# theblackcat102/edgedict

Measured on AMD Instinct MI355X. Metric: utterances/sec (E6D2, 15 s audio), higher is better.
Workload: dtype bf16; 1 GPU; E6D2 full training step (dither+log-mel+stack3+SpecAugment masks -> 6x1024 LSTM encoder, 2x time reduction -> 2x256 LSTM prediction net -> joint 640 -> RNN-T loss -> backward -> grad all-reduce -> Adam); 64 x 15 s utterances per GPU, U=64, V=2048, ragged lengths; lattice [64,201,65,2048]; global_batch=64, parallelism=dp1

## Files before the change

### edgedict_amd/config.py

```python
import os

import torch

_NAMES = {"fp32": torch.float32, "float32": torch.float32, "f32": torch.float32,
          "bf16": torch.bfloat16, "bfloat16": torch.bfloat16}


def _parse(x):
    if isinstance(x, torch.dtype):
        if x not in (torch.float32, torch.bfloat16):
            raise ValueError("compute dtype must be float32 or bfloat16")
        return x
    try:
        return _NAMES[str(x).lower()]
    except KeyError:
        raise ValueError("unknown compute dtype %r (use 'fp32' or 'bf16')" % (x,))


FORCE_GENERIC_LSTM = False

USE_ENCODER_STACK = os.environ.get("EDGEDICT_ENCODER_STACK", "1") != "0"

DEFER_WEIGHT_GRADS = os.environ.get("EDGEDICT_DEFER_DW", "1") != "0"
FUSED_DB2 = os.environ.get("EDGEDICT_FUSED_DB2", "1") != "0"

DECODER_ON_AUX_STREAM = os.environ.get("EDGEDICT_DECODER_AUX", "1") != "0"

DECODER_ENQUEUE_FIRST = os.environ.get("EDGEDICT_DECODER_FIRST", "0") != "0"

PACKED_LATTICE = os.environ.get("EDGEDICT_PACKED_LATTICE", "1") != "0"

FUSED_LSE = os.environ.get("EDGEDICT_FUSED_LSE", "1") != "0"

BAND_LATTICE = os.environ.get("EDGEDICT_BAND_LATTICE", "0") != "0"

STREAM_ENCODER_STEP = os.environ.get("EDGEDICT_STREAM_ENCODER_STEP", "1") != "0"
STREAM_STEP_MAX_ROWS_SHORT = int(os.environ.get("EDGEDICT_STREAM_STEP_MAX_ROWS_SHORT", "4096"))
STREAM_FAST_CHUNK = os.environ.get("EDGEDICT_STREAM_FAST_CHUNK", "1") != "0"
STREAM_STEP_MAX_ROWS = int(os.environ.get("EDGEDICT_STREAM_STEP_MAX_ROWS", "16"))

STACK_MIN_FRAMES = int(os.environ.get("EDGEDICT_STACK_MIN_FRAMES", "24"))

_state = {"dtype": _parse(os.environ.get("EDGEDICT_DTYPE", "fp32")), "epoch": 0}


def set_compute_dtype(x):
    _state["dtype"] = _parse(x)


def get_compute_dtype():
    return _state["dtype"]


def bump_param_epoch():
    _state["epoch"] += 1


def param_epoch():
    return _state["epoch"]
```

### edgedict_amd/csrc/elementwise.hip

```cpp
#include <cstdlib>
#include "common.hpp"

namespace {

template <typename TS, typename TD>
__global__ void cast_kernel(const TS* __restrict__ s, TD* __restrict__ d, long long n) {
    for (long long i = (long long)blockIdx.x * blockDim.x + threadIdx.x; i < n;
         i += (long long)gridDim.x * blockDim.x)
        ElemIO<TD>::store(d + i, ElemIO<TS>::load(s + i));
}

template <typename TS, typename TD>
__global__ __launch_bounds__(256) void transpose_kernel(const TS* __restrict__ s,
                                                        TD* __restrict__ d, int R, int C) {
    __shared__ float tile[32][33];
    const int tx = threadIdx.x & 31, ty = threadIdx.x >> 5;
    const int c0 = blockIdx.x * 32, r0 = blockIdx.y * 32;
#pragma unroll
    for (int i = 0; i < 4; ++i) {
        const int r = r0 + ty + i * 8, c = c0 + tx;
        tile[ty + i * 8][tx] = (r < R && c < C) ? ElemIO<TS>::load(s + (long long)r * C + c) : 0.f;
    }
    __syncthreads();
#pragma unroll
// ... 311 lines not shown
#pragma unroll
            for (int e = 0; e < 8; ++e) usum[i][e] = 0.f;
        for (int t = t0 + wave; t < t1; t += 4) {
            const int lo = max(0, bd[2 * t]), hi = min(U1 - 1, bd[2 * t + 1]);
            const long long r0 = ro[t];
            const bool ok = hi >= lo && r0 >= 0 && r0 + (hi - lo) < rows;
            const long long base = (r0 - lo) * J + j0;
            float tsum[8] = {0.f, 0.f, 0.f, 0.f, 0.f, 0.f, 0.f, 0.f};
#pragma unroll
            for (int i = 0; i < JB_NU; ++i) {
                const int u = ubase + uc + ug + 8 * i;
                if (ok && u >= lo && u <= hi && jlive) {
                    float h[8], g[8];
                    Load8<T>::ld(hid + base + (long long)u * J, h);
                    Load8<T>::ld(dhid + base + (long long)u * J, g);
#pragma unroll
                    for (int e = 0; e < 8; ++e) {
                        const float dp = g[e] * (1.f - h[e] * h[e]);
                        tsum[e] += dp;
                        usum[i][e] += dp;
                    }
                }
            }
#pragma unroll
            for (int e = 0; e < 8; ++e) {
                tsum[e] += __shfl_xor(tsum[e], 8, 64);
                tsum[e] += __shfl_xor(tsum[e], 16, 64);
                tsum[e] += __shfl_xor(tsum[e], 32, 64);
            }
            if (ug == 0 && jlive) {
                float* de = dE1 + ((long long)b * Tn + t) * J + j0;
                if (uc == 0) {
                    *reinterpret_cast<float4*>(de) = make_float4(tsum[0], tsum[1], tsum[2], tsum[3]);
                    *reinterpret_cast<float4*>(de + 4) = make_float4(tsum[4], tsum[5], tsum[6], tsum[7]);
                } else {
#pragma unroll
                    for (int e = 0; e < 8; ++e) de[e] += tsum[e];
                }
            }
        }
        if (span <= 0) break;
        if (uc > 0) __syncthreads();
        if (wave >= 2) {
#pragma unroll
            for (int i = 0; i < JB_NU; ++i) {
                red[wave - 2][i][0][lane] = make_float4(usum[i][0], usum[i][1], usum[i][2], usum[i][3]);
                red[wave - 2][i][1][lane] = make_float4(usum[i][4], usum[i][5], usum[i][6], usum[i][7]);
            }
        }
        __syncthreads();
        if (wave < 2) {
#pragma unroll
            for (int i = 0; i < JB_NU; ++i) {
                const float4 p = red[wave][i][0][lane], q = red[wave][i][1][lane];
                usum[i][0] += p.x; usum[i][1] += p.y; usum[i][2] += p.z; usum[i][3] += p.w;
                usum[i][4] += q.x; usum[i][5] += q.y; usum[i][6] += q.z; usum[i][7] += q.w;
            }
        }
        __syncthreads();
        if (wave == 1) {
#pragma unroll
            for (int i = 0; i < JB_NU; ++i) {
                red[0][i][0][lane] = make_float4(usum[i][0], usum[i][1], usum[i][2], usum[i][3]);
                red[0][i][1][lane] = make_float4(usum[i][4], usum[i][5], usum[i][6], usum[i][7]);
            }
        }
        __syncthreads();
        if (wave == 0 && jlive) {
#pragma unroll
            for (int i = 0; i < JB_NU; ++i) {
                const int u = ubase + uc + ug + 8 * i;
                if (u > uend) continue;
                const float4 p = red[0][i][0][lane], q = red[0][i][1][lane];
                float* dd = dD1 + ((long long)b * U1 + u) * J + j0;
                atomicAdd(dd + 0, usum[i][0] + p.x); atomicAdd(dd + 1, usum[i][1] + p.y);
                atomicAdd(dd + 2, usum[i][2] + p.z); atomicAdd(dd + 3, usum[i][3] + p.w);
                atomicAdd(dd + 4, usum[i][4] + q.x); atomicAdd(dd + 5, usum[i][5] + q.y);
                atomicAdd(dd + 6, usum[i][6] + q.z); atomicAdd(dd + 7, usum[i][7] + q.w);
            }
        }
    }
}

__global__ void adam_kernel(float* __restrict__ p, const float* __restrict__ g,
                            float* __restrict__ m, float* __restrict__ v, long long n, float lr,
                            float b1, float b2, float omb1, float omb2, float eps, float bc1, float bc2,
                            float weight_decay, float grad_scale_host,
                            const float* __restrict__ grad_scale,
                            bf16_t* __restrict__ p_bf16, const unsigned* __restrict__ skip) {
    if (skip && *skip != 0u) return;
    const float gs = grad_scale_host * (grad_scale ? *grad_scale : 1.f);
    const float step = lr / bc1;
    const float inv_sqrt_bc2 = rsqrtf(bc2);
    for (long long i = (long long)blockIdx.x * blockDim.x + threadIdx.x; i < n;
         i += (long long)gridDim.x * blockDim.x) {
        float gi = g[i] * gs;
        float pi = p[i];
        if (weight_decay != 0.f) gi += weight_decay * pi;
        const float mi = b1 * m[i] + omb1 * gi;
        const float vi = b2 * v[i] + omb2 * gi * gi;
        m[i] = mi;
        v[i] = vi;
        pi -= step * mi / (sqrtf(vi) * inv_sqrt_bc2 + eps);
        p[i] = pi;
        if (p_bf16) p_bf16[i] = f32_to_bf16(pi);
    }
}

__global__ void guard_fetch_kernel(const unsigned* words, int n, unsigned* scratch) {
    if (threadIdx.x == 0) {
        unsigned any = 0u;
        for (int k = 0; k < n; ++k) any |= __hip_atomic_load(words + k, __ATOMIC_RELAXED, __HIP_MEMORY_SCOPE_SYSTEM);
        *scratch = any;
    }
}

__global__ __launch_bounds__(256) void sumsq_kernel(const float* __restrict__ x, long long n,
                                                    float* __restrict__ out) {
    __shared__ float part[4];
    float a = 0.f;
    for (long long i = (long long)blockIdx.x * blockDim.x + threadIdx.x; i < n;
         i += (long long)gridDim.x * blockDim.x)
        a += x[i] * x[i];
    a = wave_sum(a);
    if ((threadIdx.x & 63) == 0) part[threadIdx.x >> 6] = a;
    __syncthreads();
    if (threadIdx.x == 0) atomicAdd(out, part[0] + part[1] + part[2] + part[3]);
}
__global__ void clip_coef_kernel(const float* sumsq, float max_norm, float pre_scale, float* coef,
                                 float* norm_out) {
    const float nrm = sqrtf(*sumsq) * pre_scale;
    if (norm_out) *norm_out = nrm;
    *coef = fminf(1.f, max_norm / (nrm + 1e-6f));
}

template <typename T>
__global__ __launch_bounds__(256) void log_softmax_rows_kernel(const T* __restrict__ x, long long ldx,
                                                               float* __restrict__ y, int N) {
    const int r = blockIdx.x, tid = threadIdx.x, lane = tid & 63, wave = tid >> 6;
    const T* xr = x + (long long)r * ldx;
    __shared__ float part[4];
    float m = -INFINITY;
    for (int i = tid; i < N; i += 256) m = fmaxf(m, ElemIO<T>::load(xr + i));
    m = wave_max(m);
    if (lane == 0) part[wave] = m;
    __syncthreads();
    m = fmaxf(fmaxf(part[0], part[1]), fmaxf(part[2], part[3]));
    __syncthreads();
    float se = 0.f;
    for (int i = tid; i < N; i += 256) se += expf(ElemIO<T>::load(xr + i) - m);
    se = wave_sum(se);
    if (lane == 0) part[wave] = se;
    __syncthreads();
    const float logs = logf((part[0] + part[1]) + (part[2] + part[3]));
    float* yr = y + (long long)r * N;
    for (int i = tid; i < N; i += 256) yr[i] = (ElemIO<T>::load(xr + i) - m) - logs;
}
template <typename T>
__global__ __launch_bounds__(256) void log_softmax_rows_bwd_kernel(const float* __restrict__ y,
                                                                   const float* __restrict__ dy, long long lddy,
                                                                   T* __restrict__ dx, int N) {
    const int r = blockIdx.x, tid = threadIdx.x, lane = tid & 63, wave = tid >> 6;
    const float* yr = y + (long long)r * N;
    const float* dyr = dy + (long long)r * lddy;
    __shared__ float part[4];
    float a = 0.f;
// ... 172 lines not shown
    if (B == 0 || T == 0 || (n_t == 0 && n_f == 0)) return ED_OK;
    ED_CHECK_ARG(x, "spec_mask: null pointer");
    hipLaunchKernelGGL(spec_mask_kernel, dim3(ed_grid_for((long long)B * T * F, 256 * 4, 256 * 16)),
                       dim3(256), 0, (hipStream_t)stream_, x, B, T, F, t_iv, n_t, f_iv, n_f);
    ED_CHECK_LAUNCH("spec_mask");
    return ED_OK;
}

static int joint_hidden_fwd_impl(int dtype, const void* E1, const void* D1, void* hid, int B, int T,
                                 int U1, int J, const int32_t* act_lens, const int32_t* label_lens,
                                 const long long* pk_off, void* stream_) {
    ED_CHECK_ARG(dtype == ED_F32 || dtype == ED_BF16, "joint_hidden_fwd: bad dtype");
    ED_CHECK_ARG(B > 0 && T > 0 && U1 > 0 && J > 0, "joint_hidden_fwd: bad shape");
    const int vec = dtype == ED_F32 ? 4 : 8;
    ED_CHECK_ARG(J % vec == 0, "joint_hidden_fwd: joint size %d must be a multiple of %d", J, vec);
    ED_CHECK_ARG(E1 && D1 && hid, "joint_hidden_fwd: null pointer");
    hipStream_t s = (hipStream_t)stream_;
    ED_CHECK_ARG(J / vec <= 256, "joint_hidden_fwd: joint size %d too large", J);
    const int grid = ed_grid_for((long long)B * T, 1, 256 * 64);
    if (dtype == ED_F32)
        hipLaunchKernelGGL(joint_hidden_fwd<float>, dim3(grid), dim3(256), 0, s, (const float*)E1, (const float*)D1, (float*)hid, B, T, U1, J, act_lens, label_lens, pk_off);
    else
        hipLaunchKernelGGL(joint_hidden_fwd<bf16_t>, dim3(grid), dim3(256), 0, s, (const bf16_t*)E1, (const bf16_t*)D1, (bf16_t*)hid, B, T, U1, J, act_lens, label_lens, pk_off);
    ED_CHECK_LAUNCH("joint_hidden_fwd");
    return ED_OK;
}

extern "C" int edgedict_joint_hidden_fwd(int dtype, const void* E1, const void* D1, void* hid,
                                         int B, int T, int U1, int J, void* stream_) {
    return joint_hidden_fwd_impl(dtype, E1, D1, hid, B, T, U1, J, nullptr, nullptr, nullptr, stream_);
}

extern "C" int edgedict_joint_hidden_fwd_packed(int dtype, const void* E1, const void* D1, void* hid,
                                                const int32_t* act_lens, const int32_t* label_lens,
                                                const long long* row_offsets, int B, int T, int U1,
                                                int J, void* stream_) {
    ED_CHECK_ARG(act_lens && label_lens && row_offsets, "joint_hidden_fwd_packed: null lengths/offsets");
    return joint_hidden_fwd_impl(dtype, E1, D1, hid, B, T, U1, J, act_lens, label_lens, row_offsets, stream_);
}

static int joint_hidden_bwd_impl(int dtype, const void* dhid, const void* hid, float* dE1, float* dD1,
                                 int B, int T, int U1, int J, const int32_t* act_lens,
                                 const int32_t* label_lens, const long long* pk_off, void* stream_) {
    ED_CHECK_ARG(dtype == ED_F32 || dtype == ED_BF16, "joint_hidden_bwd: bad dtype");
    ED_CHECK_ARG(B > 0 && T > 0 && U1 > 0 && J > 0, "joint_hidden_bwd: bad shape");
    ED_CHECK_ARG(dhid && hid && dE1 && dD1, "joint_hidden_bwd: null pointer");
    hipStream_t s = (hipStream_t)stream_;
    hipError_t e = hipMemsetAsync(dD1, 0, (size_t)B * U1 * J * sizeof(float), s);
    if (e != hipSuccess) {
        ed_set_error("joint_hidden_bwd: memset failed: %s", hipGetErrorString(e));
        return ED_ERR_LAUNCH;
    }
    ED_CHECK_ARG(J % 8 == 0, "joint_hidden_bwd: joint size %d must be a multiple of 8", J);
    const int jblocks = (J + 63) / 64;
    static const int wg_target = [] { const char* e = getenv("EDGEDICT_JHB_WGS"); return e && atoi(e) > 0 ? atoi(e) : 1280; }();
    int tslabs = (wg_target + B * jblocks - 1) / (B * jblocks);
    if (tslabs > (T + 7) / 8) tslabs = (T + 7) / 8;
    if (tslabs < 1) tslabs = 1;
    const int tpb = (T + tslabs - 1) / tslabs;
    tslabs = (T + tpb - 1) / tpb;
    dim3 grid(jblocks, B, tslabs);
    if (dtype == ED_F32)
        hipLaunchKernelGGL(joint_hidden_bwd<float>, grid, dim3(256), 0, s, (const float*)dhid, (const float*)hid, dE1, dD1, B, T, U1, J, tpb, act_lens, label_lens, pk_off);
    else
        hipLaunchKernelGGL(joint_hidden_bwd<bf16_t>, grid, dim3(256), 0, s, (const bf16_t*)dhid, (const bf16_t*)hid, dE1, dD1, B, T, U1, J, tpb, act_lens, label_lens, pk_off);
    ED_CHECK_LAUNCH("joint_hidden_bwd");
    return ED_OK;
}

extern "C" int edgedict_joint_hidden_bwd(int dtype, const void* dhid, const void* hid, float* dE1,
                                         float* dD1, int B, int T, int U1, int J, void* stream_) {
    return joint_hidden_bwd_impl(dtype, dhid, hid, dE1, dD1, B, T, U1, J, nullptr, nullptr, nullptr, stream_);
}

extern "C" int edgedict_joint_hidden_bwd_packed(int dtype, const void* dhid, const void* hid,
                                                float* dE1, float* dD1, const int32_t* act_lens,
                                                const int32_t* label_lens,
                                                const long long* row_offsets, int B, int T, int U1,
                                                int J, void* stream_) {
    ED_CHECK_ARG(act_lens && label_lens && row_offsets, "joint_hidden_bwd_packed: null lengths/offsets");
    return joint_hidden_bwd_impl(dtype, dhid, hid, dE1, dD1, B, T, U1, J, act_lens, label_lens, row_offsets, stream_);
}

extern "C" int edgedict_joint_hidden_fwd_band(int dtype, const void* E1, const void* D1, void* hid, const int32_t* band,
                                              const long long* row_off, long long rows, int B, int T, int U1, int J,
                                              void* stream_) {
    ED_CHECK_ARG(dtype == ED_F32 || dtype == ED_BF16, "joint_hidden_fwd_band: bad dtype");
    ED_CHECK_ARG(B > 0 && T > 0 && U1 > 0 && J > 0 && rows >= 0, "joint_hidden_fwd_band: bad shape");
    const int vec = dtype == ED_F32 ? 4 : 8;
    ED_CHECK_ARG(J % vec == 0, "joint_hidden_fwd_band: joint size %d must be a multiple of %d", J, vec);
    ED_CHECK_ARG(J / vec <= 256, "joint_hidden_fwd_band: joint size %d too large", J);
    if (rows == 0) return ED_OK;
    ED_CHECK_ARG(E1 && D1 && hid && band && row_off, "joint_hidden_fwd_band: null pointer");
    hipStream_t s = (hipStream_t)stream_;
    const int grid = ed_grid_for((long long)B * T, 1, 256 * 64);
    if (dtype == ED_F32)
        hipLaunchKernelGGL(joint_hidden_fwd_band<float>, dim3(grid), dim3(256), 0, s, (const float*)E1, (const float*)D1, (float*)hid, B, T, U1, J, band, row_off, rows);
    else
        hipLaunchKernelGGL(joint_hidden_fwd_band<bf16_t>, dim3(grid), dim3(256), 0, s, (const bf16_t*)E1, (const bf16_t*)D1, (bf16_t*)hid, B, T, U1, J, band, row_off, rows);
    ED_CHECK_LAUNCH("joint_hidden_fwd_band");
    return ED_OK;
}

extern "C" int edgedict_joint_hidden_bwd_band(int dtype, const void* dhid, const void* hid, float* dE1, float* dD1,
                                              const int32_t* band, const long long* row_off, long long rows, int B, int T,
                                              int U1, int J, void* stream_) {
    ED_CHECK_ARG(dtype == ED_F32 || dtype == ED_BF16, "joint_hidden_bwd_band: bad dtype");
    ED_CHECK_ARG(B > 0 && T > 0 && U1 > 0 && J > 0 && rows >= 0, "joint_hidden_bwd_band: bad shape");
    ED_CHECK_ARG((rows == 0 || (dhid && hid)) && dE1 && dD1 && band && row_off, "joint_hidden_bwd_band: null pointer");
    ED_CHECK_ARG(J % 8 == 0, "joint_hidden_bwd_band: joint size %d must be a multiple of 8", J);
    hipStream_t s = (hipStream_t)stream_;
    hipError_t e = hipMemsetAsync(dD1, 0, (size_t)B * U1 * J * sizeof(float), s);
    if (e != hipSuccess) {
        ed_set_error("joint_hidden_bwd_band: memset failed: %s", hipGetErrorString(e));
        return ED_ERR_LAUNCH;
    }
    const int jblocks = (J + 63) / 64;
    int tslabs = (1280 + B * jblocks - 1) / (B * jblocks);
    if (tslabs > (T + 7) / 8) tslabs = (T + 7) / 8;
    if (tslabs < 1) tslabs = 1;
    const int tpb = (T + tslabs - 1) / tslabs;
    tslabs = (T + tpb - 1) / tpb;
    dim3 grid(jblocks, B, tslabs);
    if (dtype == ED_F32)
        hipLaunchKernelGGL(joint_hidden_bwd_band<float>, grid, dim3(256), 0, s, (const float*)dhid, (const float*)hid, dE1, dD1, B, T, U1, J, tpb, band, row_off, rows);
    else
        hipLaunchKernelGGL(joint_hidden_bwd_band<bf16_t>, grid, dim3(256), 0, s, (const bf16_t*)dhid, (const bf16_t*)hid, dE1, dD1, B, T, U1, J, tpb, band, row_off, rows);
    ED_CHECK_LAUNCH("joint_hidden_bwd_band");
    return ED_OK;
}

extern "C" int edgedict_adam_step_guarded(float* p, const float* g, float* m, float* v, long long n,
                                          float lr, float beta1, float beta2, float eps, int step,
                                          float weight_decay, float grad_scale_host,
                                          const float* grad_scale, void* p_bf16,
                                          const unsigned* skip_words, int n_skip, unsigned* guard_scratch,
                                          void* stream_) {
    ED_CHECK_ARG(n >= 0 && step >= 1, "adam_step: bad size/step");
    if (n == 0) return ED_OK;
    ED_CHECK_ARG(p && g && m && v, "adam_step: null pointer");
    ED_CHECK_ARG(n_skip >= 0 && n_skip <= 16 && (n_skip == 0 || (skip_words && guard_scratch)),
                 "adam_step_guarded: bad guard words / scratch");
    if (n_skip > 0) {
        hipLaunchKernelGGL(guard_fetch_kernel, dim3(1), dim3(64), 0, (hipStream_t)stream_, skip_words, n_skip, guard_scratch);
        ED_CHECK_LAUNCH("guard_fetch_kernel");
    }
    const double b1d = nearbyint((double)beta1 * 1e7) / 1e7, b2d = nearbyint((double)beta2 * 1e7) / 1e7;
    const float omb1 = (float)(1.0 - b1d), omb2 = (float)(1.0 - b2d);
    const float bc1 = (float)(1.0 - pow(b1d, (double)step));
    const float bc2 = (float)(1.0 - pow(b2d, (double)step));
    hipLaunchKernelGGL(adam_kernel, dim3(ed_grid_for(n, 256 * 4, 256 * 8)), dim3(256), 0,
                       (hipStream_t)stream_, p, g, m, v, n, lr, beta1, beta2, omb1, omb2, eps, bc1, bc2,
                       weight_decay, grad_scale_host, grad_scale, (bf16_t*)p_bf16, n_skip > 0 ? guard_scratch : nullptr);
    ED_CHECK_LAUNCH("adam_step");
    return ED_OK;
}

extern "C" int edgedict_adam_step(float* p, const float* g, float* m, float* v, long long n,
                                  float lr, float beta1, float beta2, float eps, int step,
                                  float weight_decay, float grad_scale_host,
                                  const float* grad_scale, void* p_bf16, void* stream_) {
    return edgedict_adam_step_guarded(p, g, m, v, n, lr, beta1, beta2, eps, step, weight_decay, grad_scale_host,
                                      grad_scale, p_bf16, nullptr, 0, nullptr, stream_);
}

extern "C" int edgedict_grad_clip_coef(const float* g, long long n, float max_norm,
// ... 54 lines not shown
```

### edgedict_amd/models.py

```python
import math
import weakref

import torch
from torch import nn

from . import config, encoder_stack, ops, side
from . import _lib
from ._lib import require_cuda
from .loss import _RNNTLossFn
from .tokenizer import BOS, NUL, PAD

F32 = torch.float32


class _WeightCache:
    def __init__(self):
        self._store = {}

    def get(self, p, dtype, transposed=False):
        key = (id(p), dtype, transposed)
        ver = (p.data_ptr(), p._version, config.param_epoch())
        hit = self._store.get(key)
        if hit is not None and hit[0] == ver and hit[2]() is p:
            return hit[1]
        dead = [k for k, v in self._store.items() if v[2]() is None]
        for k in dead:
            del self._store[k]
        src = p.detach()
        if not src.is_contiguous():
            src = src.contiguous()
        if transposed == "lstm_fwd":
            t = ops.lstm_pack_weights(src, True, False)[0]
        elif transposed == "lstm_bwd":
            t = ops.lstm_pack_weights(src, False, True)[1]
        elif transposed:
            t = ops.transpose(src, dtype)
        elif dtype == src.dtype:
            t = src
        else:
            t = ops.cast(src, dtype)
        if t is not src and t.is_cuda:
            from . import side
            for s in (torch.cuda.current_stream(t.device), side.peek(t.device)):
                if s is not None:
                    t.record_stream(s)
        self._store[key] = (ver, t, weakref.ref(p))
        return t

    def clear(self):
        self._store.clear()


WEIGHTS = _WeightCache()


def _lstm_fast(cd, H):
    return cd == torch.bfloat16 and H % 32 == 0 and not config.FORCE_GENERIC_LSTM


def _to_cd(x, cd):
    if x.dtype == cd:
        return x.contiguous()
    if x.dtype not in (torch.float32, torch.bfloat16):
        x = x.float()
    return ops.cast(x.contiguous(), cd)


def _state(t):
    if t is None:
        return None
    t = t.detach()
    if t.dtype != F32:
        t = ops.cast(t.contiguous(), F32)
    return t.contiguous()


class _InputNormFn(torch.autograd.Function):

    @staticmethod
    def forward(ctx, xs, gamma, beta, cd):
        x = _to_cd(xs, cd)
        y, mean, rstd = ops.layernorm_fwd(x, None, gamma.detach(), beta.detach(), 1)
# ... 381 lines not shown
        tables = (plan.band, plan.row_off, plan.row_tu, plan.cells)
        if config.FUSED_LSE and cd == torch.bfloat16 and J >= 128 and J % 64 == 0 and V % 8 == 0 and M >= 256:
            slots = (V + 63) // 64
            parts = torch.empty(M, slots, 2, dtype=F32, device=dev)
            logits = torch.empty(M, V, dtype=cd, device=dev)
            ops.fire("before_logits_gemm")
            with ops.timed("joint_logits_gemm"):
                _lib.call("gemm_nt_lse", hid, ops._ll(J), w2c, ops._ll(J), logits, ops._ll(V), M, V, J,
                          b2.detach(), parts)
            with ops.timed("rnnt_loss_fwd"):
                _lib.call("rnnt_loss_forward_band_parts", logits, labels, al_d, ll_d, win_lo, win_hi, *tables,
                          B, T, U1, V, int(blank), costs, reduced, 1.0 / B, ws, parts, slots)
        else:
            with ops.timed("joint_logits_gemm"):
                logits = ops.gemm(hid, w2c, bias=b2.detach())
            _lib.call("rnnt_loss_forward_band", logits, _lib.dtype_code(cd), labels, al_d, ll_d, win_lo, win_hi, *tables,
                      B, T, U1, V, int(blank), costs, reduced, 1.0 / B, ws)
        ops.LAST["joint_costs"] = costs
        ctx.save_for_backward(enc2, dec2, w1, w2, hid, logits, labels, al_d, ll_d, ws)
        return reduced

    @staticmethod
    def _backward_band(ctx, gout):
        plan = ctx.plan
        cd, B, T, U1, P, P2, J, V, M, blank = ctx.cfg
        tail = (None,) * 10
        if M == 0:
            enc2, dec2, w1, w2 = ctx.saved_tensors
            with side.WeightGrads(ctx, 2, (w1, ctx.b1, w2, ctx.b2)) as wg:
                for i in range(4):
                    wg.zero(i)
            ops.mark("joint_bwd:exit")
            return (torch.zeros(B, T, P, dtype=enc2.dtype, device=enc2.device),
                    torch.zeros(B, U1, P2, dtype=dec2.dtype, device=dec2.device), *wg.grads, *tail)
        enc2, dec2, w1, w2, hid, logits, labels, al_d, ll_d, ws = ctx.saved_tensors
        dl = torch.empty_like(logits)
        gscale = gout.contiguous().float()
        w1c = WEIGHTS.get(w1, cd)
        w2t = WEIGHTS.get(w2, cd, transposed=True)
        dE1 = torch.empty(B, T, J, dtype=F32, device=dl.device)
        dD1 = torch.empty(B, U1, J, dtype=F32, device=dl.device)
        cs_rows = _lib.load().edgedict_rnnt_grad_colsum_rows(_lib.dtype_code(cd), B, T, U1, V) if config.FUSED_DB2 else 0
        db2_parts = torch.empty(cs_rows, V, dtype=F32, device=dl.device) if cs_rows > 0 else None
        rows = (plan.row_off, plan.row_tu, plan.cells)
        with ops.timed("rnnt_grad"):
            if db2_parts is not None:
                _lib.call("rnnt_loss_backward_band_colsum", logits, _lib.dtype_code(cd), dl, labels, al_d, ll_d, *rows,
                          B, T, U1, V, blank, ws, 1.0 / B, gscale, 0, db2_parts, ctx.fastemit_lambda)
            else:
                _lib.call("rnnt_loss_backward_band", logits, _lib.dtype_code(cd), dl, labels, al_d, ll_d, *rows,
                          B, T, U1, V, blank, ws, 1.0 / B, gscale, 0, ctx.fastemit_lambda)
        del logits
        with ops.timed("joint_dhid_gemm"):
            dhid = ops.gemm(dl, w2t)
        with ops.timed("joint_hidden_bwd"):
            _lib.call("joint_hidden_bwd_band", _lib.dtype_code(cd), dhid, hid, dE1, dD1, plan.band, plan.row_off,
                      ops._ll(M), B, T, U1, J)
        del dhid
        dE1c = ops.cast(dE1, cd).view(B * T, J)
        dD1c = ops.cast(dD1, cd).view(B * U1, J)
        denc = ops.gemm(dE1c, w1c[:, :P].t()).view(B, T, P)
        ddec = ops.gemm(dD1c, w1c[:, P:].t()).view(B, U1, P2)
        with side.WeightGrads(ctx, 2, (w1, ctx.b1, w2, ctx.b2), dl, hid, dE1c, dD1c, dD1, enc2, dec2, db2_parts) as wg:
            wg.gemm(2, dl.t(), hid.t(), split_k=ops.pick_split_k(V, J, M), aux=dict(split_k=8, max_wg_per_cu=2))
            wg.colsum(3, dl if db2_parts is None else db2_parts)
            wg.gemm(0, dE1c.t(), enc2.t(), cols=slice(None, P), split_k=ops.pick_split_k(J, P, B * T))
            wg.gemm(0, dD1c.t(), dec2.t(), cols=slice(P, None), split_k=ops.pick_split_k(J, P2, B * U1))
            wg.colsum(1, dD1.view(B * U1, J))
        ops.mark("joint_bwd:exit")
        return (denc, ddec, *wg.grads, *tail)

    @staticmethod
    def backward(ctx, gout):
        ops.mark("joint_bwd:enter")
        if ctx.plan is not None:
            return _JointLossFn._backward_band(ctx, gout)
        enc2, dec2, w1, w2, hid, logits, labels, al_d, ll_d, off_d, ws = ctx.saved_tensors
        cd, B, T, U1, P, P2, J, V, M, blank = ctx.cfg
        dl = torch.empty_like(logits)
        gscale = gout.contiguous().float()
        gs_host, gs_stride = (1.0, 1) if ctx.row_costs else (1.0 / B, 0)
        w1c = WEIGHTS.get(w1, cd)
        w2t = WEIGHTS.get(w2, cd, transposed=True)
        dE1 = torch.empty(B, T, J, dtype=F32, device=dl.device)
        dD1 = torch.empty(B, U1, J, dtype=F32, device=dl.device)
        cs_rows = _lib.load().edgedict_rnnt_grad_colsum_rows(_lib.dtype_code(cd), B, T, U1, V) if config.FUSED_DB2 else 0
        db2_parts = torch.empty(cs_rows, V, dtype=F32, device=dl.device) if cs_rows > 0 else None
        lam = ctx.fastemit_lambda
        with ops.timed("rnnt_grad"):
            if ctx.restricted:
                if db2_parts is not None:
                    _lib.call("rnnt_loss_backward_packed_colsum_ar", logits, _lib.dtype_code(cd), dl, labels, al_d,
                              ll_d, off_d, B, T, U1, V, blank, ws, gs_host, gscale, gs_stride, db2_parts, lam)
                else:
                    _lib.call("rnnt_loss_backward_packed_ar", logits, _lib.dtype_code(cd), dl, labels, al_d, ll_d,
                              off_d, B, T, U1, V, blank, ws, gs_host, gscale, gs_stride, lam)
            elif lam != 0.0:
                if db2_parts is not None:
                    _lib.call("rnnt_loss_backward_packed_colsum_fe", logits, _lib.dtype_code(cd), dl, labels, al_d,
                              ll_d, off_d, B, T, U1, V, blank, ws, gs_host, gscale, gs_stride, db2_parts, lam)
                else:
                    _lib.call("rnnt_loss_backward_packed_fe", logits, _lib.dtype_code(cd), dl, labels, al_d, ll_d,
                              off_d, B, T, U1, V, blank, ws, gs_host, gscale, gs_stride, lam)
            elif db2_parts is not None:
                _lib.call("rnnt_loss_backward_packed_colsum", logits, _lib.dtype_code(cd), dl, labels, al_d, ll_d,
                          off_d, B, T, U1, V, blank, ws, gs_host, gscale, gs_stride, db2_parts)
            else:
                _lib.call("rnnt_loss_backward_packed", logits, _lib.dtype_code(cd), dl, labels, al_d, ll_d,
                          off_d, B, T, U1, V, blank, ws, gs_host, gscale, gs_stride)
        del logits
        with ops.timed("joint_dhid_gemm"):
            dhid = ops.gemm(dl, w2t)
        with ops.timed("joint_hidden_bwd"):
            _lib.call("joint_hidden_bwd_packed", _lib.dtype_code(cd), dhid, hid, dE1, dD1, al_d, ll_d,
                      off_d, B, T, U1, J)
        del dhid
        dE1c = ops.cast(dE1, cd).view(B * T, J)
        dD1c = ops.cast(dD1, cd).view(B * U1, J)
        denc = ops.gemm(dE1c, w1c[:, :P].t()).view(B, T, P)
        ddec = ops.gemm(dD1c, w1c[:, P:].t()).view(B, U1, P2)
        with side.WeightGrads(ctx, 2, (w1, ctx.b1, w2, ctx.b2), dl, hid, dE1c, dD1c, dD1, enc2, dec2, db2_parts) as wg:
            wg.gemm(2, dl.t(), hid.t(), split_k=ops.pick_split_k(V, J, M), aux=dict(split_k=8, max_wg_per_cu=2))
            wg.colsum(3, dl if db2_parts is None else db2_parts)
            wg.gemm(0, dE1c.t(), enc2.t(), cols=slice(None, P), split_k=ops.pick_split_k(J, P, B * T))
            wg.gemm(0, dD1c.t(), dec2.t(), cols=slice(P, None), split_k=ops.pick_split_k(J, P2, B * U1))
            wg.colsum(1, dD1.view(B * U1, J))
        ops.mark("joint_bwd:exit")
        return (denc, ddec, *wg.grads, None, None, None, None, None, None, None, None, None, None)


class TimeReduction(nn.Module):

    def __init__(self, reduction_factor=2):
        super().__init__()
        self.reduction_factor = reduction_factor


class _LayerNormParams(nn.Module):
    def __init__(self, size, eps=1e-5):
        super().__init__()
        self.normalized_shape = (size,)
        self.eps = eps
        self.weight = nn.Parameter(torch.ones(size))
        self.bias = nn.Parameter(torch.zeros(size))


class _LinearParams(nn.Module):
    def __init__(self, in_features, out_features):
        super().__init__()
        self.in_features, self.out_features = in_features, out_features
        self.weight = nn.Parameter(torch.empty(out_features, in_features))
        self.bias = nn.Parameter(torch.empty(out_features))
        nn.init.kaiming_uniform_(self.weight, a=math.sqrt(5))
        bound = 1.0 / math.sqrt(in_features)
        nn.init.uniform_(self.bias, -bound, bound)


class _LSTMParams(nn.Module):

    def __init__(self, input_size, hidden_size, num_layers=1, dropout=0.0):
        super().__init__()
        self.input_size, self.hidden_size = input_size, hidden_size
        self.num_layers, self.dropout = num_layers, dropout
        k = 1.0 / math.sqrt(hidden_size)
        for layer in range(num_layers):
            i = input_size if layer == 0 else hidden_size
            for name, shape in (("weight_ih", (4 * hidden_size, i)),
                                ("weight_hh", (4 * hidden_size, hidden_size)),
                                ("bias_ih", (4 * hidden_size,)),
                                ("bias_hh", (4 * hidden_size,))):
                p = nn.Parameter(torch.empty(*shape).uniform_(-k, k))
                setattr(self, "%s_l%d" % (name, layer), p)

    def layer(self, k):
        return tuple(getattr(self, "%s_l%d" % (n, k))
                     for n in ("weight_ih", "weight_hh", "bias_ih", "bias_hh"))

    def flatten_parameters(self):
        pass


class ResLayerNormLSTM(nn.Module):

    def __init__(self, input_size, hidden_size, num_layers, dropout=0,
                 time_reductions=[1], reduction_factor=2):
        super().__init__()
        if reduction_factor != 2:
            raise ValueError("only reduction_factor=2 is implemented (the reference default)")
        self.dropout = dropout
        self.hidden_size = hidden_size
        self.lstms = nn.ModuleList()
        self.projs = nn.ModuleList()
        self.reductions = []
        for i in range(num_layers):
            self.lstms.append(_LSTMParams(input_size, hidden_size, 1))
            proj = [_LayerNormParams(hidden_size)]
            if i in time_reductions:
                proj.append(TimeReduction(reduction_factor))
            self.reductions.append(2 if i in time_reductions else 1)
            input_size = hidden_size
            self.projs.append(nn.Sequential(*proj))
# ... 810 lines not shown
```

### include/edgedict_hip.h

```cpp
#ifndef EDGEDICT_HIP_H
#define EDGEDICT_HIP_H

#include <stddef.h>
#include <stdint.h>

#ifdef __cplusplus
extern "C" {
#endif

#define EDGEDICT_ABI_VERSION 2

#define ED_OK 0
#define ED_ERR_INVALID (-1)
#define ED_ERR_LAUNCH (-2)

#define ED_F32 0
#define ED_BF16 1

const char* edgedict_last_error(void);
int edgedict_abi_version(void);

size_t edgedict_rnnt_workspace_bytes(int B, int T, int U1);
int edgedict_rnnt_loss_forward(const void* acts, int acts_dtype, const int32_t* labels,
                               const int32_t* act_lens, const int32_t* label_lens, int B, int T,
// ... 219 lines not shown
#define EDGEDICT_STACK_SERIAL 1
#define EDGEDICT_STACK_DW_AT_END 2
#define EDGEDICT_STACK_ACCUM_GRADS 8
#define EDGEDICT_STACK_INFERENCE 64
#define EDGEDICT_STACK_SIDE_STREAM_PER_LAYER 4

typedef struct edgedict_stack_desc {
    int B, H, L;
    int chunk;
    int lag;
    int split_k;
    int flags;
    float eps;
    const edgedict_stack_layer_t* layers;
    const void* x;
    int x_dtype, T0, I0;
    const float* in_gamma;
    const float* in_beta;
    float* in_mean;
    float* in_rstd;
    const float* h0;
    const float* c0;
    void* out;
    const void* dout;
    float* d_in_gamma;
    float* d_in_beta;
    void* ws;
    size_t ws_bytes;
    void (*grads_final)(int layer, void* user);
    void* grads_final_user;
} edgedict_stack_desc_t;

size_t edgedict_stack_struct_bytes(int which);
void* edgedict_aux_stream(int which);
int edgedict_streams_busy(unsigned* mask);
size_t edgedict_stack_workspace_bytes(const edgedict_stack_desc_t* desc);
int edgedict_stack_pack_weights(const float* w_ih, const float* w_hh, const float* b_ih,
                                const float* b_hh, int H, int I, void* wih_p, void* wih_t,
                                float* bias_p, void* whh_f, void* whh_b, void* stream);
int edgedict_stack_pack_sk(const float* w_hh, int H, void* whh_s, void* stream);
int edgedict_stack_wsr_error(void);
void* edgedict_stack_error_words(int host);
int edgedict_stack_wsr_set_trace(void* device_buffer);
int edgedict_stack_forward(const edgedict_stack_desc_t* desc, void* stream);
int edgedict_stack_last_timing(int backward, float* ms, int* launches);
int edgedict_stack_last_mode(int backward, int* kind, int* steps_per_launch);
int edgedict_stack_time_launches(int on);
int edgedict_stack_launch_times(int backward, float* sum_ms, int* launches);
int edgedict_stack_launch_stamps(int backward, unsigned long long* out, int max_launches, int* launches);
int edgedict_stack_schedule(const edgedict_stack_desc_t* d, int backward, int32_t* step_launch,
                            int32_t* chunk_enqueued, int32_t* n_launches, int32_t* max_slots);
int edgedict_stack_schedule_events(const edgedict_stack_desc_t* d, int32_t* events, int capacity, int32_t* n_events);
int edgedict_stack_tail_mode(int bits);
int edgedict_stack_backward(const edgedict_stack_desc_t* desc, void* stream);

int edgedict_cast(int src_dtype, const void* src, int dst_dtype, void* dst, long long n,
                  void* stream);
int edgedict_transpose(int src_dtype, const void* src, int dst_dtype, void* dst, int R, int C,
                       void* stream);
int edgedict_colsum(int dtype, const void* x, long long ld, float* out, long long M, int N,
                    void* stream);
int edgedict_embedding_fwd(int out_dtype, int emb_dtype, const int32_t* tokens, int tok_stride,
                           const void* emb, void* out, int B, int Uout, int E, int V,
                           int prepend_bos, int bos, void* stream);
int edgedict_embedding_bwd(int dtype, const int32_t* tokens, int tok_stride, const void* dout,
                           float* demb, int B, int Uout, int E, int V, int prepend_bos, int bos,
                           int pad, void* stream);
int edgedict_dropout(int dtype, const void* x, void* y, long long n, float p, unsigned seed,
                     void* stream);
int edgedict_spec_mask(float* x, int B, int T, int F, const int32_t* t_iv, int n_t,
                       const int32_t* f_iv, int n_f, void* stream);
int edgedict_joint_hidden_fwd(int dtype, const void* E1, const void* D1, void* hid, int B, int T,
                              int U1, int J, void* stream);
int edgedict_joint_hidden_bwd(int dtype, const void* dhid, const void* hid, float* dE1,
                              float* dD1, int B, int T, int U1, int J, void* stream);
int edgedict_joint_hidden_fwd_packed(int dtype, const void* E1, const void* D1, void* hid,
                                     const int32_t* act_lens, const int32_t* label_lens,
                                     const long long* row_offsets, int B, int T, int U1, int J,
                                     void* stream);
int edgedict_joint_hidden_bwd_packed(int dtype, const void* dhid, const void* hid, float* dE1,
                                     float* dD1, const int32_t* act_lens, const int32_t* label_lens,
                                     const long long* row_offsets, int B, int T, int U1, int J,
                                     void* stream);
int edgedict_joint_hidden_fwd_band(int dtype, const void* E1, const void* D1, void* hid, const int32_t* band,
                                   const long long* row_off, long long rows, int B, int T, int U1, int J, void* stream);
int edgedict_joint_hidden_bwd_band(int dtype, const void* dhid, const void* hid, float* dE1, float* dD1,
                                   const int32_t* band, const long long* row_off, long long rows, int B, int T, int U1,
                                   int J, void* stream);

int edgedict_adam_step(float* p, const float* g, float* m, float* v, long long n, float lr,
                       float beta1, float beta2, float eps, int step, float weight_decay,
                       float grad_scale_host, const float* grad_scale, void* p_bf16, void* stream);
int edgedict_adam_step_guarded(float* p, const float* g, float* m, float* v, long long n, float lr,
                               float beta1, float beta2, float eps, int step, float weight_decay,
                               float grad_scale_host, const float* grad_scale, void* p_bf16,
                               const unsigned* skip_words, int n_skip, unsigned* guard_scratch,
                               void* stream);
int edgedict_grad_clip_coef(const float* g, long long n, float max_norm, float pre_scale,
                            float* sumsq_ws, float* coef, float* norm_out, void* stream);
int edgedict_debug_footprint(float* buf, long long n_floats, int workgroups, int passes, void* stream);

int edgedict_dither(float* wave, long long wave_stride, int B, int N, const int32_t* lengths,
                    float amplitude, unsigned seed, void* stream);
int edgedict_fbank_forward(const float* wave, long long wave_stride, int B, int N,
                           const int32_t* lengths, const float* window, const float* twiddle,
                           const float* fb, const int32_t* fb_range, int n_fft, int win_lo,
                           int win_hi, int hop, int n_mels, float preemph, int do_log, void* out,
                           int out_dtype, long long o_b, long long o_group, long long o_k,
                           long long o_m, int stack, int frames_out, void* stream);
int edgedict_fbank_forward_masked(const float* wave, long long wave_stride, int B, int N,
                                  const int32_t* seq_len, const float* window,
                                  const float* twiddle, const float* fb, const int32_t* fb_range,
                                  int n_fft, int win_lo, int win_hi, int hop, int n_mels,
                                  float preemph, int do_log, float* out, long long o_b,
                                  long long o_m, int frames_out, int copies, long long o_copy,
                                  int normalize, int n_signal, void* stream);

size_t edgedict_greedy_workspace_bytes(int dtype, int B, int J, int V, int E, int L, int H, int P2);
int edgedict_greedy_decode(int dtype, const void* E1, long long e_row_stride,
                           long long e_frame_stride, int B, int T, int J, const void* W1d,
                           long long ldw1, const float* b1, int P2, const void* W2,
                           const float* b2, int V, const void* emb, int emb_dtype, int E, int L,
                           const void* const* w_ih, const void* const* w_hh,
                           const float* const* b_ih, const float* const* b_hh, int H,
                           const void* Wp, const float* bp, float* h_state, float* c_state,
                           void* dec_out, int blank, int unk, int32_t* tokens_out, int tok_stride,
                           float* score, void* workspace, void* stream);
int edgedict_decode_fused_ok(int dtype, int emb_dtype, int J, int V, int E, int H, int P2);

int edgedict_gru_forward(int dtype, void* G, void* Hprev, void* Y, void* HN, const void* Whh,
                         const float* b_hh, const float* h0, float* hN, int B, int T, int H,
                         void* stream);
int edgedict_gru_backward(int dtype, void* G, void* DH, const void* dY, const void* Hprev,
                          const void* HN, const void* WhhT, float* dh_ws, int B, int T, int H,
                          void* stream);

int edgedict_conv_out_frames(int Tin, int k, int s);
int edgedict_conv_im2col(int in_dtype, int out_dtype, const void* x, void* cols, int B, int Tin, int C,
                         int k, int s, void* stream);
int edgedict_conv_col2im(int dtype, const void* dcols, void* dx, int B, int Tin, int C, int k, int s,
                         void* stream);
int edgedict_gelu_groupnorm_fwd(int dtype, const void* y, const float* gamma, const float* beta,
                                void* out, float* mean, float* rstd, int B, int T, int C, float eps,
                                void* stream);
size_t edgedict_gelu_groupnorm_bwd_workspace_bytes(int B, int T, int C);
int edgedict_gelu_groupnorm_bwd(int dtype, const void* y, const void* dout, const float* gamma,
                                const float* mean, const float* rstd, void* dy, float* dgamma,
                                float* dbeta, void* workspace, int B, int T, int C, void* stream);

long long edgedict_blaslt_calls(void);

size_t edgedict_stream_encoder_workspace_bytes(int B, int T, int I0, int H, int L);
int edgedict_stream_encoder_step(const void* xs, int x_dtype, int B, int T, int I0, int H, int L,
                                 const float* in_gamma, const float* in_beta, const void* const* w_ih,
                                 const void* const* w_hh, const float* const* b_ih, const float* const* b_hh,
                                 const float* const* ln_gamma, const float* const* ln_beta, const int* reduce,
                                 float* h_state, float* c_state, void* out, int* T_out, void* workspace,
                                 void* stream);

struct edgedict_beam_lm_t;
struct edgedict_beam_bias_t;
typedef struct edgedict_search_net_t {
    int dtype;
    int J;
    const void* W1d;
    long long ldw1;
// ... 213 lines not shown
```

Before: 3417 utterances/s.

## Replace joint hidden backward atomics with slab partial sums and fused bf16 casts

Adds a new joint-hidden backward kernel that splits each utterance's time range into S slabs. Each slab writes its label-position partial sums to a workspace, and a finish kernel reduces them, replacing the float atomicAdd accumulation into dD1. The kernel writes dE1 directly in bf16, and the finish kernel also writes the bf16 copy of dD1, which removes the separate cast kernels and the fp32 dE1 buffer. Loads use AMD buffer-load intrinsics with out-of-range offsets for dead lanes. The cost is an extra workspace allocation of B*S*U1*J floats plus one more launch for the finish pass.

```diff
diff --git a/edgedict_amd/config.py b/edgedict_amd/config.py
--- a/edgedict_amd/config.py
+++ b/edgedict_amd/config.py
@@ -32,6 +32,8 @@
 
 FUSED_LSE = os.environ.get("EDGEDICT_FUSED_LSE", "1") != "0"
 
+JHB_PARTS = os.environ.get("EDGEDICT_JHB_PARTS", "1") != "0"
+
 BAND_LATTICE = os.environ.get("EDGEDICT_BAND_LATTICE", "0") != "0"
 
 STREAM_ENCODER_STEP = os.environ.get("EDGEDICT_STREAM_ENCODER_STEP", "1") != "0"
diff --git a/edgedict_amd/csrc/elementwise.hip b/edgedict_amd/csrc/elementwise.hip
--- a/edgedict_amd/csrc/elementwise.hip
+++ b/edgedict_amd/csrc/elementwise.hip
@@ -417,6 +417,218 @@
     }
 }
 
+typedef __attribute__((ext_vector_type(4))) unsigned jb_u32x4_t;
+constexpr unsigned JB_OFF_DEAD = 0x80000000u;
+__device__ __forceinline__ __amdgpu_buffer_rsrc_t jb_rsrc(const void* p, unsigned bytes) {
+    const unsigned long long a = (unsigned long long)p;
+    const unsigned lo = __builtin_amdgcn_readfirstlane((unsigned)a);
+    const unsigned hi = __builtin_amdgcn_readfirstlane((unsigned)(a >> 32));
+    return __builtin_amdgcn_make_buffer_rsrc((void*)(((unsigned long long)hi << 32) | lo), 0,
+                                             (int)__builtin_amdgcn_readfirstlane(bytes), 0x00020000);
+}
+template <typename T> struct Raw8;
+template <> struct Raw8<bf16_t> {
+    jb_u32x4_t v;
+    __device__ __forceinline__ void ld(__amdgpu_buffer_rsrc_t r, unsigned off) {
+        v = __builtin_amdgcn_raw_buffer_load_b128(r, off, 0, 0);
+    }
+    __device__ __forceinline__ void get(float (&o)[8]) const {
+        ElemIO<bf16_t>::cvt_vec(make_uint4(v.x, v.y, v.z, v.w), o);
+    }
+};
+template <> struct Raw8<float> {
+    jb_u32x4_t a, b;
+    __device__ __forceinline__ void ld(__amdgpu_buffer_rsrc_t r, unsigned off) {
+        a = __builtin_amdgcn_raw_buffer_load_b128(r, off, 0, 0);
+        b = __builtin_amdgcn_raw_buffer_load_b128(r, off + 16u, 0, 0);
+    }
+    __device__ __forceinline__ void get(float (&o)[8]) const {
+        o[0] = __uint_as_float(a.x); o[1] = __uint_as_float(a.y); o[2] = __uint_as_float(a.z); o[3] = __uint_as_float(a.w);
+        o[4] = __uint_as_float(b.x); o[5] = __uint_as_float(b.y); o[6] = __uint_as_float(b.z); o[7] = __uint_as_float(b.w);
+    }
+};
+template <typename T> constexpr int jb_batch() { return sizeof(T) == 2 ? JB_NU : 3; }
+static_assert(JB_NU % jb_batch<float>() == 0, "label positions in whole batches");
+
+template <typename T> struct Store8;
+template <> struct Store8<bf16_t> {
+    __device__ static __forceinline__ void st(bf16_t* p, const float (&o)[8]) { ElemIO<bf16_t>::store_vec(p, o); }
+};
+template <> struct Store8<float> {
+    __device__ static __forceinline__ void st(float* p, const float (&o)[8]) {
+        *reinterpret_cast<float4*>(p) = make_float4(o[0], o[1], o[2], o[3]);
+        *reinterpret_cast<float4*>(p + 4) = make_float4(o[4], o[5], o[6], o[7]);
+    }
+};
+
+__device__ __forceinline__ void jb_combine_waves(float4 (&red)[2][JB_NU][2][64], float (&usum)[JB_NU][8], int wave,
+                                                 int lane, bool again) {
+    if (again) __syncthreads();
+    if (wave >= 2) {
+#pragma unroll
+        for (int i = 0; i < JB_NU; ++i) {
+            red[wave - 2][i][0][lane] = make_float4(usum[i][0], usum[i][1], usum[i][2], usum[i][3]);
+            red[wave - 2][i][1][lane] = make_float4(usum[i][4], usum[i][5], usum[i][6], usum[i][7]);
+        }
+    }
+    __syncthreads();
+    if (wave < 2) {
+#pragma unroll
+        for (int i = 0; i < JB_NU; ++i) {
+            const float4 p = red[wave][i][0][lane], q = red[wave][i][1][lane];
+            usum[i][0] += p.x; usum[i][1] += p.y; usum[i][2] += p.z; usum[i][3] += p.w;
+            usum[i][4] += q.x; usum[i][5] += q.y; usum[i][6] += q.z; usum[i][7] += q.w;
+        }
+    }
+    __syncthreads();
+    if (wave == 1) {
+#pragma unroll
+        for (int i = 0; i < JB_NU; ++i) {
+            red[0][i][0][lane] = make_float4(usum[i][0], usum[i][1], usum[i][2], usum[i][3]);
+            red[0][i][1][lane] = make_float4(usum[i][4], usum[i][5], usum[i][6], usum[i][7]);
+        }
+    }
+    __syncthreads();
+    if (wave == 0) {
+#pragma unroll
+        for (int i = 0; i < JB_NU; ++i) {
+            const float4 p = red[0][i][0][lane], q = red[0][i][1][lane];
+            usum[i][0] += p.x; usum[i][1] += p.y; usum[i][2] += p.z; usum[i][3] += p.w;
+            usum[i][4] += q.x; usum[i][5] += q.y; usum[i][6] += q.z; usum[i][7] += q.w;
+        }
+    }
+}
+
+template <typename T>
+__device__ __forceinline__ void jb_frame_out(T* __restrict__ dE1c, float* __restrict__ erow, long long at, int pass,
+                                             int passes, float (&tsum)[8]) {
+    if (passes > 1) {
+        float* er = erow + at;
+        if (pass > 0) {
+            const float4 a = *reinterpret_cast<const float4*>(er), c = *reinterpret_cast<const float4*>(er + 4);
+            tsum[0] = a.x + tsum[0]; tsum[1] = a.y + tsum[1]; tsum[2] = a.z + tsum[2]; tsum[3] = a.w + tsum[3];
+            tsum[4] = c.x + tsum[4]; tsum[5] = c.y + tsum[5]; tsum[6] = c.z + tsum[6]; tsum[7] = c.w + tsum[7];
+        }
+        if (pass < passes - 1) {
+            Store8<float>::st(er, tsum);
+            return;
+        }
+    }
+    Store8<T>::st(dE1c + at, tsum);
+}
+
+template <typename T>
+__global__ __launch_bounds__(256, 2) void joint_hidden_bwd_parts(const T* __restrict__ dhid, const T* __restrict__ hid,
+                                                              T* __restrict__ dE1c, float* __restrict__ parts,
+                                                              float* __restrict__ erow, int B, int Tn, int U1, int J,
+                                                              int S, const int32_t* __restrict__ act_lens,
+                                                              const int32_t* __restrict__ label_lens,
+                                                              const long long* __restrict__ pk_off) {
+    __shared__ float4 red[2][JB_NU][2][64];
+    const int lane = threadIdx.x & 63, wave = __builtin_amdgcn_readfirstlane(threadIdx.x >> 6);
+    const int jv = lane & 7, ug = lane >> 3;
+    const int j0 = blockIdx.x * 64 + jv * 8;
+    const int b = blockIdx.y, s = blockIdx.z;
+    const bool jlive = j0 < J;
+    const int Tb = min(max(act_lens[b], 0), Tn);
+    const int Ulim = min(max(label_lens[b], 0) + 1, U1);
+    const long long rbase = pk_off[b];
+    const int Fb = (Tb + S - 1) / S;
+    const int t0 = min(Tb, s * Fb), t1 = min(Tb, t0 + Fb);
+    {
+        const int pad = Tn - Tb, Pb = (pad + S - 1) / S;
+        const int z0 = Tb + min(pad, s * Pb), z1 = min(Tn, z0 + Pb);
+        float zero[8] = {0.f, 0.f, 0.f, 0.f, 0.f, 0.f, 0.f, 0.f};
+        if (jlive)
+            for (int t = z0 + (threadIdx.x >> 3); t < z1; t += 32)
+                Store8<T>::st(dE1c + ((long long)b * Tn + t) * J + j0, zero);
+    }
+    const int passes = (U1 + JB_UCHUNK - 1) / JB_UCHUNK;
+    const unsigned fbytes = (unsigned)Ulim * (unsigned)J * (unsigned)sizeof(T);
+    for (int pass = 0; pass < passes; ++pass) {
+        const int uc = pass * JB_UCHUNK;
+        const unsigned at0 = ((unsigned)(uc + ug) * (unsigned)J + (unsigned)j0) * (unsigned)sizeof(T);
+        const unsigned step = 8u * (unsigned)J * (unsigned)sizeof(T);
+        float usum[JB_NU][8];
+#pragma unroll
+        for (int i = 0; i < JB_NU; ++i)
+#pragma unroll
+            for (int e = 0; e < 8; ++e) usum[i][e] = 0.f;
+        for (int t = t0 + wave; t < t1; t += 4) {
+            const long long frame = (rbase + (long long)t * Ulim) * J;
+            const __amdgpu_buffer_rsrc_t fh = jb_rsrc(hid + frame, fbytes), fg = jb_rsrc(dhid + frame, fbytes);
+            float tsum[8] = {0.f, 0.f, 0.f, 0.f, 0.f, 0.f, 0.f, 0.f};
+#pragma unroll
+            for (int i0 = 0; i0 < JB_NU; i0 += jb_batch<T>()) {
+                Raw8<T> rh[jb_batch<T>()], rg[jb_batch<T>()];
+#pragma unroll
+                for (int k = 0; k < jb_batch<T>(); ++k) {
+                    const unsigned at = uc + ug + 8 * (i0 + k) < Ulim && jlive ? at0 + (unsigned)(i0 + k) * step : JB_OFF_DEAD;
+                    rh[k].ld(fh, at);
+                    rg[k].ld(fg, at);
+                }
+#pragma unroll
+                for (int k = 0; k < jb_batch<T>(); ++k) {
+                    float h[8], g[8];
+                    rh[k].get(h);
+                    rg[k].get(g);
+#pragma unroll
+                    for (int e = 0; e < 8; ++e) {
+                        const float x = __builtin_fmaf(-h[e], h[e], 1.f);
+                        tsum[e] = __builtin_fmaf(g[e], x, tsum[e]);
+                        usum[i0 + k][e] = __builtin_fmaf(g[e], x, usum[i0 + k][e]);
+                    }
+                }
+            }
+#pragma unroll
+            for (int e = 0; e < 8; ++e) {
+                tsum[e] += __shfl_xor(tsum[e], 8, 64);
+                tsum[e] += __shfl_xor(tsum[e], 16, 64);
+                tsum[e] += __shfl_xor(tsum[e], 32, 64);
+            }
+            if (ug == 0 && jlive) jb_frame_out<T>(dE1c, erow, ((long long)b * Tn + t) * J + j0, pass, passes, tsum);
+        }
+        jb_combine_waves(red, usum, wave, lane, pass > 0);
+        if (wave == 0 && jlive) {
+            float* pp = parts + (((long long)b * S + s) * U1) * J + j0;
+#pragma unroll
+            for (int i = 0; i < JB_NU; ++i) {
+                const int u = uc + ug + 8 * i;
+                if (u < U1) Store8<float>::st(pp + (long long)u * J, usum[i]);
+            }
+        }
+    }
+}
+
+__device__ __forceinline__ void jb_store4(float* p, const float4& a) { *reinterpret_cast<float4*>(p) = a; }
+__device__ __forceinline__ void jb_store4(bf16_t* p, const float4& a) {
+    *reinterpret_cast<uint2*>(p) = make_uint2(f32x2_to_bf16x2(a.x, a.y), f32x2_to_bf16x2(a.z, a.w));
+}
+
+template <typename T>
+__global__ __launch_bounds__(256) void joint_dD1_finish(const float* __restrict__ parts, float* __restrict__ dD1,
+                                                        T* __restrict__ dD1c, int B, int U1, int J, int S,
+                                                        const int32_t* __restrict__ label_lens) {
+    const int q = J / 4;
+    const long long n = (long long)B * U1 * q, slab = (long long)U1 * J;
+    for (long long i = (long long)blockIdx.x * blockDim.x + threadIdx.x; i < n; i += (long long)gridDim.x * blockDim.x) {
+        const int bu = (int)(i / q), j = (int)(i - (long long)bu * q) * 4;
+        const int b = bu / U1, u = bu - b * U1;
+        float4 a = make_float4(0.f, 0.f, 0.f, 0.f);
+        if (u <= label_lens[b]) {
+            const float* p = parts + ((long long)b * S * U1 + u) * J + j;
+            a = *reinterpret_cast<const float4*>(p);
+            for (int s = 1; s < S; ++s) {
+                const float4 c = *reinterpret_cast<const float4*>(p + s * slab);
+                a.x += c.x; a.y += c.y; a.z += c.z; a.w += c.w;
+            }
+        }
+        const long long at = (long long)bu * J + j;
+        *reinterpret_cast<float4*>(dD1 + at) = a;
+        jb_store4(dD1c + at, a);
+    }
+}
+
 __global__ void adam_kernel(float* __restrict__ p, const float* __restrict__ g,
                             float* __restrict__ m, float* __restrict__ v, long long n, float lr,
                             float b1, float b2, float omb1, float omb2, float eps, float bc1, float bc2,
@@ -755,6 +967,57 @@
     return joint_hidden_bwd_impl(dtype, dhid, hid, dE1, dD1, B, T, U1, J, act_lens, label_lens, row_offsets, stream_);
 }
 
+static int jhb_slabs(int B, int J) {
+    const int forced = ed_env_now("EDGEDICT_JHB_SLABS", 0);
+    const long long cols = (long long)B * ((J + 63) / 64);
+    const long long S = forced > 0 ? forced : (1280 + cols - 1) / cols;
+    return S > 16 ? 16 : S < 1 ? 1 : (int)S;
+}
+
+static size_t jhb_parts_elems(int B, int U1, int J) { return (size_t)B * jhb_slabs(B, J) * U1 * J; }
+
+extern "C" size_t edgedict_joint_hidden_bwd_workspace_bytes(int dtype, int B, int T, int U1, int J) {
+    (void)dtype;
+    if (B <= 0 || T <= 0 || U1 <= 0 || J <= 0) return 0;
+    return sizeof(float) * (jhb_parts_elems(B, U1, J) + (U1 > JB_UCHUNK ? (size_t)B * T * J : 0));
+}
+
+extern "C" int edgedict_joint_hidden_bwd_packed_parts(int dtype, const void* dhid, const void* hid, void* dE1c,
+                                                      float* dD1, void* dD1c, void* workspace, size_t workspace_bytes,
+                                                      const int32_t* act_lens, const int32_t* label_lens,
+                                                      const long long* row_offsets, int B, int T, int U1, int J,
+                                                      void* stream_) {
+    ED_CHECK_ARG(dtype == ED_F32 || dtype == ED_BF16, "joint_hidden_bwd_packed_parts: bad dtype");
+    ED_CHECK_ARG(B > 0 && T > 0 && U1 > 0 && J > 0, "joint_hidden_bwd_packed_parts: bad shape");
+    ED_CHECK_ARG(B <= 65535, "joint_hidden_bwd_packed_parts: batch %d above the grid's 65535", B);
+    ED_CHECK_ARG(J % 8 == 0, "joint_hidden_bwd_packed_parts: joint size %d must be a multiple of 8", J);
+    ED_CHECK_ARG((long long)U1 * J * 4 < (1ll << 31), "joint_hidden_bwd_packed_parts: U1 * J = %lld too large", (long long)U1 * J);
+    ED_CHECK_ARG(dhid && hid && dE1c && dD1 && dD1c && workspace, "joint_hidden_bwd_packed_parts: null pointer");
+    ED_CHECK_ARG(act_lens && label_lens && row_offsets, "joint_hidden_bwd_packed_parts: null lengths/offsets");
+    ED_CHECK_ARG(workspace_bytes >= edgedict_joint_hidden_bwd_workspace_bytes(dtype, B, T, U1, J),
+                 "joint_hidden_bwd_packed_parts: workspace of %zu bytes, %zu needed", workspace_bytes,
+                 edgedict_joint_hidden_bwd_workspace_bytes(dtype, B, T, U1, J));
+    ED_CHECK_ARG(((uintptr_t)dhid | (uintptr_t)hid | (uintptr_t)dE1c | (uintptr_t)dD1 | (uintptr_t)dD1c |
+                  (uintptr_t)workspace) % 16 == 0, "joint_hidden_bwd_packed_parts: pointers must be 16-byte aligned");
+    hipStream_t s = (hipStream_t)stream_;
+    const int S = jhb_slabs(B, J);
+    float* parts = (float*)workspace;
+    float* erow = U1 > JB_UCHUNK ? parts + jhb_parts_elems(B, U1, J) : nullptr;
+    dim3 grid((J + 63) / 64, B, S);
+    const int fgrid = ed_grid_for((long long)B * U1 * (J / 4), 256, 256 * 16);
+    if (dtype == ED_F32) {
+        hipLaunchKernelGGL(joint_hidden_bwd_parts<float>, grid, dim3(256), 0, s, (const float*)dhid, (const float*)hid, (float*)dE1c, parts, erow, B, T, U1, J, S, act_lens, label_lens, row_offsets);
+        ED_CHECK_LAUNCH("joint_hidden_bwd_parts");
+        hipLaunchKernelGGL(joint_dD1_finish<float>, dim3(fgrid), dim3(256), 0, s, parts, dD1, (float*)dD1c, B, U1, J, S, label_lens);
+    } else {
+        hipLaunchKernelGGL(joint_hidden_bwd_parts<bf16_t>, grid, dim3(256), 0, s, (const bf16_t*)dhid, (const bf16_t*)hid, (bf16_t*)dE1c, parts, erow, B, T, U1, J, S, act_lens, label_lens, row_offsets);
+        ED_CHECK_LAUNCH("joint_hidden_bwd_parts");
+        hipLaunchKernelGGL(joint_dD1_finish<bf16_t>, dim3(fgrid), dim3(256), 0, s, parts, dD1, (bf16_t*)dD1c, B, U1, J, S, label_lens);
+    }
+    ED_CHECK_LAUNCH("joint_dD1_finish");
+    return ED_OK;
+}
+
 extern "C" int edgedict_joint_hidden_fwd_band(int dtype, const void* E1, const void* D1, void* hid, const int32_t* band,
                                               const long long* row_off, long long rows, int B, int T, int U1, int J,
                                               void* stream_) {
diff --git a/edgedict_amd/models.py b/edgedict_amd/models.py
--- a/edgedict_amd/models.py
+++ b/edgedict_amd/models.py
@@ -1,3 +1,4 @@
+import ctypes
 import math
 import weakref
 
@@ -545,7 +546,6 @@
         gs_host, gs_stride = (1.0, 1) if ctx.row_costs else (1.0 / B, 0)
         w1c = WEIGHTS.get(w1, cd)
         w2t = WEIGHTS.get(w2, cd, transposed=True)
-        dE1 = torch.empty(B, T, J, dtype=F32, device=dl.device)
         dD1 = torch.empty(B, U1, J, dtype=F32, device=dl.device)
         cs_rows = _lib.load().edgedict_rnnt_grad_colsum_rows(_lib.dtype_code(cd), B, T, U1, V) if config.FUSED_DB2 else 0
         db2_parts = torch.empty(cs_rows, V, dtype=F32, device=dl.device) if cs_rows > 0 else None
@@ -574,12 +574,23 @@
         del logits
         with ops.timed("joint_dhid_gemm"):
             dhid = ops.gemm(dl, w2t)
-        with ops.timed("joint_hidden_bwd"):
-            _lib.call("joint_hidden_bwd_packed", _lib.dtype_code(cd), dhid, hid, dE1, dD1, al_d, ll_d,
-                      off_d, B, T, U1, J)
-        del dhid
-        dE1c = ops.cast(dE1, cd).view(B * T, J)
-        dD1c = ops.cast(dD1, cd).view(B * U1, J)
+        if config.JHB_PARTS and cd == torch.bfloat16:
+            dE1c = torch.empty(B * T, J, dtype=cd, device=dl.device)
+            dD1c = torch.empty(B * U1, J, dtype=cd, device=dl.device)
+            nws = _lib.load().edgedict_joint_hidden_bwd_workspace_bytes(_lib.dtype_code(cd), B, T, U1, J)
+            jws = torch.empty(nws, dtype=torch.uint8, device=dl.device)
+            with ops.timed("joint_hidden_bwd"):
+                _lib.call("joint_hidden_bwd_packed_parts", _lib.dtype_code(cd), dhid, hid, dE1c, dD1, dD1c, jws,
+                          ctypes.c_size_t(nws), al_d, ll_d, off_d, B, T, U1, J)
+            del dhid, jws
+        else:
+            dE1 = torch.empty(B, T, J, dtype=F32, device=dl.device)
+            with ops.timed("joint_hidden_bwd"):
+                _lib.call("joint_hidden_bwd_packed", _lib.dtype_code(cd), dhid, hid, dE1, dD1, al_d, ll_d,
+                          off_d, B, T, U1, J)
+            del dhid
+            dE1c = ops.cast(dE1, cd).view(B * T, J)
+            dD1c = ops.cast(dD1, cd).view(B * U1, J)
         denc = ops.gemm(dE1c, w1c[:, :P].t()).view(B, T, P)
         ddec = ops.gemm(dD1c, w1c[:, P:].t()).view(B, U1, P2)
         with side.WeightGrads(ctx, 2, (w1, ctx.b1, w2, ctx.b2), dl, hid, dE1c, dD1c, dD1, enc2, dec2, db2_parts) as wg:
diff --git a/include/edgedict_hip.h b/include/edgedict_hip.h
--- a/include/edgedict_hip.h
+++ b/include/edgedict_hip.h
@@ -325,6 +325,11 @@
                                      float* dD1, const int32_t* act_lens, const int32_t* label_lens,
                                      const long long* row_offsets, int B, int T, int U1, int J,
                                      void* stream);
+size_t edgedict_joint_hidden_bwd_workspace_bytes(int dtype, int B, int T, int U1, int J);
+int edgedict_joint_hidden_bwd_packed_parts(int dtype, const void* dhid, const void* hid, void* dE1c, float* dD1,
+                                           void* dD1c, void* workspace, size_t workspace_bytes,
+                                           const int32_t* act_lens, const int32_t* label_lens,
+                                           const long long* row_offsets, int B, int T, int U1, int J, void* stream);
 int edgedict_joint_hidden_fwd_band(int dtype, const void* E1, const void* D1, void* hid, const int32_t* band,
                                    const long long* row_off, long long rows, int B, int T, int U1, int J, void* stream);
 int edgedict_joint_hidden_bwd_band(int dtype, const void* dhid, const void* hid, float* dE1, float* dD1,
```

Result: no change. 3422 utterances/s, median of 4 (+0.1%).
